# qc-tum/TNC

Measured on NVIDIA H100. Metric: pairwise contractions/sec (effective ZGEMM TFLOP/s in zgemm_tflops), higher is better.
Workload: dtype f64

## Files before the change

tnc_b200/csrc/crt.cu:

```cuda
#include "internal.h"
#include "sm90.h"
#include <cuda.h>
#include <algorithm>
#include <cmath>
#include <cstdio>
#include <cstdlib>

namespace tncb {

constexpr int CRT_MAX_MOD = 20;
static const int kModuli[CRT_MAX_MOD] = {256, 253, 251, 249, 247, 245, 241, 239, 233, 229,
                                         227, 223, 211, 199, 197, 193, 191, 181, 179, 173};
constexpr int CRT_BT = 128;
constexpr int CRT_BKB = WG_BKB;
#ifndef CRT_RING3_STAGES
#define CRT_RING3_STAGES 3
#endif
#ifndef CRT_RING3_BK
#define CRT_RING3_BK 128
#endif
#ifndef CRT_RING4_STAGES
#define CRT_RING4_STAGES 5
#endif
#ifndef CRT_RING4_BK
// ... 65 lines not shown
    T.inv_mod[i] = 1.0 / (double)m;
    T.rho1[i] = std::ldexp((double)q, -CRT_G);
    T.rho2[i] = std::ldexp((double)rem / (double)m, -CRT_G);
  }
  T.p_scaled = (double)std::ldexp(P, -(bits_a + bits_b));
}

int crt_export_tables(int nmod, int* moduli, double* rho1, double* rho2, double* log2_product) {
  CrtTables T;
  crt_make_tables(nmod, 0, 0, T);
  for (int i = 0; i < nmod; i++) {
    if (moduli) moduli[i] = T.mod[i];
    if (rho1) rho1[i] = T.rho1[i];
    if (rho2) rho2[i] = T.rho2[i];
  }
  if (log2_product) *log2_product = crt_log2_product(nmod);
  return TNCB_OK;
}

constexpr int RES_ROWS_C = 32, RES_K_C = 128;
constexpr int kExpNonFinite = 0x7fffffff;
constexpr int kExpMin = -1000;

__device__ __forceinline__ int crt_exp_from_bits(unsigned long long bits) {
  const int field = (int)(bits >> 52) & 0x7ff;
  if (field == 0x7ff) return kExpNonFinite;
  if (field == 0) return bits == 0ull ? 0 : kExpMin;
  return max(field - 1022, kExpMin);
}

__device__ __forceinline__ void crt_tile_coord(int e, int lk, int& r, int& k) {
  const int lane = e & 31, blk = e >> 5;
  const int kb = blk & ((128 >> lk) - 1), rb = blk >> (7 - lk);
  k = (kb << lk) + (lane & ((1 << lk) - 1));
  r = (rb << (5 - lk)) + (lane >> lk);
}

__global__ void __launch_bounds__(256)
crt_rowmax_kernel(const double2* __restrict__ src, const long long* __restrict__ off_row, const long long* __restrict__ off_k,
                  long long rows, long long K, int lk, unsigned long long* __restrict__ rowmax) {
  __shared__ unsigned long long s_max[RES_ROWS_C];
  __shared__ long long s_offr[RES_ROWS_C], s_offk[RES_K_C];
  const long long row0 = (long long)blockIdx.x * RES_ROWS_C, k0 = (long long)blockIdx.y * RES_K_C;
  const int tid = threadIdx.x;
  if (tid < RES_ROWS_C) { s_max[tid] = 0ull; s_offr[tid] = row0 + tid < rows ? __ldg(off_row + row0 + tid) : -1; }
  else if (tid >= 128) { const int k = tid - 128; s_offk[k] = k0 + k < K ? __ldg(off_k + k0 + k) : -1; }
  __syncthreads();
  unsigned long long mv[RES_ROWS_C * RES_K_C / 256];
#pragma unroll
  for (int it = 0; it < RES_ROWS_C * RES_K_C / 256; it++) {
    int r, k;
    crt_tile_coord(it * 256 + tid, lk, r, k);
    const long long orow = s_offr[r], ok = s_offk[k];
    mv[it] = 0ull;
    if (orow >= 0 && ok >= 0) {
      const double2 v = __ldg(src + orow + ok);
      mv[it] = max((unsigned long long)__double_as_longlong(fabs(v.x)), (unsigned long long)__double_as_longlong(fabs(v.y)));
    }
  }
  int cur_r = -1;
  unsigned long long cur_m = 0ull;
#pragma unroll
  for (int it = 0; it < RES_ROWS_C * RES_K_C / 256; it++) {
    int r, k;
    crt_tile_coord(it * 256 + tid, lk, r, k);
    unsigned long long m = mv[it];
    for (int d = 1; d < (1 << lk); d <<= 1) m = max(m, __shfl_xor_sync(0xffffffffu, m, d));
    if (r != cur_r) {
      if (cur_m && (tid & ((1 << lk) - 1)) == 0) atomicMax(&s_max[cur_r], cur_m);
      cur_r = r; cur_m = 0ull;
    }
    cur_m = max(cur_m, m);
  }
  if (cur_m && (tid & ((1 << lk) - 1)) == 0) atomicMax(&s_max[cur_r], cur_m);
  __syncthreads();
  if (tid < RES_ROWS_C && row0 + tid < rows && s_max[tid] != 0ull) atomicMax(rowmax + row0 + tid, s_max[tid]);
}

__device__ __forceinline__ int crt_fix_byte(int s, int m) {
  if (s > 127) s -= m;
  else if (s < -128) s += m;
  return s;
}
constexpr int RES_ROWS = RES_ROWS_C, RES_K = RES_K_C, RES_RS = RES_K + RES_K / 8 + 1;
template <int COMPS, bool KARA>
__global__ void __launch_bounds__(256, 3)
crt_residue_kernel(const double2* __restrict__ src, const long long* __restrict__ off_row, const long long* __restrict__ off_k,
                   long long rows, long long K, long long rowsP, long long Kp, const unsigned long long* __restrict__ rowmax, int bits, int lk,
                   const __grid_constant__ CrtTables T, int8_t* __restrict__ planes) {
  extern __shared__ __align__(16) unsigned char res_smem_raw[];
  double2* tile = reinterpret_cast<double2*>(res_smem_raw);
  __shared__ double s_scale[RES_ROWS];
  __shared__ long long s_offr[RES_ROWS], s_offk[RES_K];
  __shared__ double s_inv[CRT_MAX_MOD];
  __shared__ int s_mod[CRT_MAX_MOD];
  const long long row0 = (long long)blockIdx.x * RES_ROWS, k0 = (long long)blockIdx.y * RES_K;
  const int tid = threadIdx.x;
  const double two_a = scalbn(1.0, bits);
  if (tid >= 64 && tid < 64 + CRT_MAX_MOD) { s_inv[tid - 64] = T.inv_mod[tid - 64]; s_mod[tid - 64] = T.mod[tid - 64]; }
  if (tid < RES_ROWS) {
    const long long r = row0 + tid;
    const int e = r < rows ? crt_exp_from_bits(rowmax[r]) : 0;
    s_scale[tid] = (e == kExpNonFinite) ? 0.0 : scalbn(1.0, -e);
    s_offr[tid] = r < rows ? __ldg(off_row + r) : -1;
  } else if (tid >= 128) {
    const int k = tid - 128;
    s_offk[k] = k0 + k < K ? __ldg(off_k + k0 + k) : -1;
  }
  __syncthreads();
  double2 vv[RES_ROWS * RES_K / 256];
#pragma unroll
  for (int it = 0; it < RES_ROWS * RES_K / 256; it++) {
    int r, k;
    crt_tile_coord(it * 256 + tid, lk, r, k);
    const long long orow = s_offr[r], ok = s_offk[k];
    vv[it] = make_double2(0.0, 0.0);
    if (orow >= 0 && ok >= 0) vv[it] = __ldg(src + orow + ok);
  }
#pragma unroll
  for (int it = 0; it < RES_ROWS * RES_K / 256; it++) {
    int r, k;
    crt_tile_coord(it * 256 + tid, lk, r, k);
    const double sc = s_scale[r];
    double2 v = vv[it];
    v.x = trunc(v.x * sc * two_a);
    v.y = trunc(v.y * sc * two_a);
    if (sc == 0.0) { v.x = 0.0; v.y = 0.0; }
    tile[r * RES_RS + k + (k >> 3)] = v;
  }
  __syncthreads();
  const double RMAGIC = 6755399441055744.0;
  const long long plane_stride = rowsP * Kp;
  const int g = tid & 31;
  const int nmod = T.nmod;
#pragma unroll 1
  for (int pass = 0; pass < RES_ROWS / 8; pass++) {
    const int r = (tid >> 5) + 8 * pass;
    if (row0 + r >= rows) return;
    double xr[4], xi[4];
    int lr[4], li[4];
#pragma unroll
    for (int j = 0; j < 4; j++) {
      const double2 v = tile[r * RES_RS + g * 4 + j + (g >> 1)];
      xr[j] = v.x; xi[j] = v.y;
      lr[j] = (int)__double2ll_rn(v.x); li[j] = (int)__double2ll_rn(v.y);
    }
    int8_t* dst = planes + (row0 + r) * Kp + k0 + g * 4;
#pragma unroll 1
    for (int i = 0; i < nmod; i++) {
      const int m = s_mod[i];
      const double inv = s_inv[i];
      uint32_t wr = 0, wi = 0, ws = 0;
#pragma unroll
      for (int j = 0; j < 4; j++) {
        const int qr = __double2loint(fma(xr[j], inv, RMAGIC));
        const int qi = __double2loint(fma(xi[j], inv, RMAGIC));
        const int rr = lr[j] - qr * m, ri = li[j] - qi * m;
        constexpr uint32_t sel[4] = {0x3214u, 0x3240u, 0x3410u, 0x4210u};
        wr = __byte_perm(wr, (uint32_t)rr, sel[j]);
        wi = __byte_perm(wi, (uint32_t)ri, sel[j]);
        if (KARA) ws = __byte_perm(ws, (uint32_t)crt_fix_byte(rr + ri, m), sel[j]);
      }
      uint32_t* d = reinterpret_cast<uint32_t*>(dst + (long long)i * (KARA ? 3 : COMPS) * plane_stride);
      const long long ps = plane_stride / 4;
      if (KARA) {
        d[0] = wr; d[ps] = wi; d[2 * ps] = ws;
      } else if (COMPS == 2) {
        d[0] = wr; d[ps] = wi;
      } else {
        d[0] = __vneg4(wi); d[ps] = wr; d[2 * ps] = wi;
      }
    }
  }
}

struct CrtGemmArgs {
  int8_t* R;
  int Np, Mp;
  int tiles_n, tiles_m, tile_m;
  int nmod, nkc, kb_per_chunk, num_kb;
  int total_items;
  int group;
  int negmod[CRT_MAX_MOD];
  int magic[CRT_MAX_MOD];
};

struct CrtItem { int mod_i, prod, kc, n0, m0; };
template <bool KARA>
__device__ __forceinline__ CrtItem crt_decode(const CrtGemmArgs& p, int item) {
  const int tiles = p.tiles_n * p.tiles_m;
  const int mk = item / tiles, t = item - mk * tiles;
  CrtItem it;
  const int mp = mk / p.nkc;
  it.kc = mk - mp * p.nkc;
  it.mod_i = KARA ? mp / 3 : mp; it.prod = KARA ? mp - it.mod_i * 3 : 0;
  const int per_band = p.group * p.tiles_m;
  const int band = t / per_band, first = band * p.group;
  const int gsize = min(p.group, p.tiles_n - first);
  const int r = t - band * per_band;
  it.n0 = (first + r % gsize) * CRT_BT;
  it.m0 = (r / gsize) * p.tile_m;
  return it;
}

template <bool KARA>
__global__ void __launch_bounds__(WG_THREADS, 1)
crt_gemm_kernel(const __grid_constant__ CUtensorMap mapB, const __grid_constant__ CUtensorMap mapA,
                const __grid_constant__ CrtGemmArgs p) {
  constexpr int STAGES = CrtRing<KARA>::STAGES, BK = CrtRing<KARA>::BK, SUB = CRT_BKB / BK;
  using Stage = typename CrtRing<KARA>::Stage;
  extern __shared__ __align__(1024) uint8_t crt_smem_raw[];
  uint8_t* smem = reinterpret_cast<uint8_t*>((reinterpret_cast<uintptr_t>(crt_smem_raw) + 1023) & ~(uintptr_t)1023);
  __shared__ uint64_t full_bar[STAGES], empty_bar[STAGES];
  const int wg = threadIdx.x >> 7, tid = threadIdx.x & 127;

  if (threadIdx.x == 0) {
    for (int s = 0; s < STAGES; s++) { wg_mbar_init(&full_bar[s], 1); wg_mbar_init(&empty_bar[s], 2); }
    asm volatile("fence.mbarrier_init.release.cluster;" ::: "memory");
  }
  __syncthreads();

  if (wg == 0) {
    wg_setmaxnreg_producer();
    if (tid != 0) return;
    int it = 0;
    for (int item = blockIdx.x; item < p.total_items; item += gridDim.x) {
      const CrtItem w = crt_decode<KARA>(p, item);
      const int kb0 = w.kc * p.kb_per_chunk, kb1 = min(p.num_kb, kb0 + p.kb_per_chunk);
      const int rowB = (KARA ? w.mod_i * 3 + w.prod : w.mod_i * 2) * p.Np + w.n0;
      const int rowA = (KARA ? w.mod_i * 3 + w.prod : w.mod_i * 3) * p.Mp + w.m0;
      for (int ks = kb0 * SUB; ks < kb1 * SUB; ks++, it++) {
        uint8_t* st = wg_produce_begin<STAGES, KARA, BK>(smem, full_bar, empty_bar, it);
        uint64_t* bar = &full_bar[it % STAGES];
        const int kx = ks * BK;
        uint8_t* a = st + Stage::A;
        wg_tma_2d(&mapB, bar, st, kx, rowB);
        if (KARA) {
          wg_tma_2d(&mapA, bar, a, kx, rowA);
          wg_tma_2d(&mapA, bar, a + Stage::TILE, kx, rowA + WG_ROWS);
        } else {
          wg_tma_2d(&mapB, bar, st + Stage::B1, kx, rowB + p.Np);
          wg_tma_2d(&mapA, bar, a, kx, rowA);
          wg_tma_2d(&mapA, bar, a + Stage::TILE, kx, rowA + p.Mp);
          wg_tma_2d(&mapA, bar, a + 2 * Stage::TILE, kx, rowA + 2 * p.Mp);
        }
      }
    }
  } else {
    wg_setmaxnreg_consumer();
    const int c = wg - 1, wq = tid >> 5, lane = tid & 31;
    const int q = lane & 3;
    const bool q0 = q & 1, q1 = q & 2;
    WgRing<STAGES, KARA, BK> ring{smem, full_bar, empty_bar};
    uint32_t acc[128];
#pragma unroll
    for (int i = 0; i < 128; i++) acc[i] = 0u;
    for (int item = blockIdx.x; item < p.total_items; item += gridDim.x) {
      const CrtItem w = crt_decode<KARA>(p, item);
      const int kb0 = w.kc * p.kb_per_chunk, kb1 = min(p.num_kb, kb0 + p.kb_per_chunk);
      bool first = true;
      for (int ks = kb0 * SUB; ks < kb1 * SUB; ks++) ring.mma_stage(acc, c, first, tid == 0);
      ring.drain(tid == 0);
      const int negm = p.negmod[w.mod_i], magic = p.magic[w.mod_i];
      int8_t* row_base[2];
#pragma unroll
      for (int h = 0; h < 2; h++) {
        const long long n = (long long)w.n0 + c * 64 + wq * 16 + (lane >> 2) + 8 * h;
        row_base[h] = KARA ? p.R + ((long long)((w.mod_i * p.nkc + w.kc) * 3 + w.prod) * p.Np + n) * p.Mp + w.m0
                           : p.R + ((long long)((w.mod_i * p.nkc + w.kc) * 2) * p.Np + n) * p.Mp + w.m0;
      }
#pragma unroll
      for (int i = 0; i < 4; i++) {
#pragma unroll
        for (int h = 0; h < 2; h++) {
          uint32_t x[4];
#pragma unroll
          for (int k = 0; k < 4; k++) {
            uint32_t u = 0;
#pragma unroll
            for (int jj = 0; jj < 2; jj++) {
#pragma unroll
              for (int e = 0; e < 2; e++) {
                const int a = (int)acc[4 * (8 * i + 2 * k + jj) + 2 * h + e];
                int t = __mulhi(a, magic) * negm + a;
                if (t > 127) t += negm;
                u |= (((uint32_t)t & 0xffu) ^ 0x80u) << (8 * (2 * jj + e));
              }
            }
            x[k] = u;
          }
          const uint32_t r0 = __shfl_xor_sync(0xffffffffu, q0 ? x[0] : x[1], 1);
          const uint32_t r1 = __shfl_xor_sync(0xffffffffu, q0 ? x[2] : x[3], 1);
          const uint32_t a0 = q0 ? r0 : x[0], a1 = q0 ? x[1] : r0;
          const uint32_t b0 = q0 ? r1 : x[2], b1 = q0 ? x[3] : r1;
          const uint32_t g0 = __shfl_xor_sync(0xffffffffu, q1 ? a0 : b0, 2);
          const uint32_t g1 = __shfl_xor_sync(0xffffffffu, q1 ? a1 : b1, 2);
          const uint32_t k0 = q1 ? b0 : a0, k1 = q1 ? b1 : a1;
          const uint32_t y0 = q1 ? g0 : k0, y1 = q1 ? g1 : k1, y2 = q1 ? k0 : g0, y3 = q1 ? k1 : g1;
          const uint4 v = make_uint4(__byte_perm(y0, y1, 0x5410), __byte_perm(y2, y3, 0x5410),
                                     __byte_perm(y0, y1, 0x7632), __byte_perm(y2, y3, 0x7632));
          const int cc = 4 * i + q;
          int8_t* dst = KARA ? row_base[h] + cc * 16
                             : row_base[h] + (i >= 2 ? (long long)p.Np * p.Mp : 0LL) + (cc & 7) * 16;
          *reinterpret_cast<uint4*>(dst) = v;
        }
      }
    }
  }
}

struct CrtReconArgs {
  const int8_t* R;
  double2* C;
  const unsigned long long* max_n;
  const unsigned long long* max_m;
  long long rows, cols, ldc;
  long long Np, Mp;
  int nkc;
};

template <bool ONE_CHUNK, bool KARA>
__global__ void __launch_bounds__(256, KARA ? 3 : 4)
crt_reconstruct_kernel(const __grid_constant__ CrtReconArgs a, const __grid_constant__ CrtTables T) {
  constexpr int NPR = KARA ? 3 : 2, RB = 8;
  const long long cols4 = a.Mp >> 2;
  const long long idx = (long long)blockIdx.x * blockDim.x + threadIdx.x;
  const long long n = idx / cols4, m4 = (idx - n * cols4) * 4;
  if (n >= a.rows || m4 >= a.cols) return;
  double s1r[4], s2r[4], s1i[4], s2i[4];
#pragma unroll
  for (int j = 0; j < 4; j++) { s1r[j] = s2r[j] = s1i[j] = s2i[j] = 0.0; }
  const long long plane = a.Np * a.Mp;
  const int8_t* base = a.R + n * a.Mp + m4;
  const double bias = 4503599627370496.0 + (KARA ? 256.0 : 128.0) * (double)a.nkc;
  const double bias_i = 4503599627370496.0 + (KARA ? 384.0 : 128.0) * (double)a.nkc;
  const int nmod = T.nmod;
#pragma unroll 1
  for (int i0 = 0; i0 < nmod; i0 += RB) {
    uint32_t w[RB][NPR];
    if (ONE_CHUNK) {
#pragma unroll
      for (int u = 0; u < RB; u++) {
        if (i0 + u < nmod) {
#pragma unroll
          for (int p = 0; p < NPR; p++) w[u][p] = __ldg(reinterpret_cast<const uint32_t*>(base + (long long)((i0 + u) * NPR + p) * plane));
        }
      }
    }
#pragma unroll
    for (int u = 0; u < RB; u++) {
      const int i = i0 + u;
      if (i >= nmod) break;
      uint32_t ur[4], ui[4];
#pragma unroll
      for (int j = 0; j < 4; j++) { ur[j] = 0; ui[j] = 0; }
      for (int c = 0; c < (ONE_CHUNK ? 1 : a.nkc); c++) {
        uint32_t x[NPR];
        if (ONE_CHUNK) {
#pragma unroll
          for (int p = 0; p < NPR; p++) x[p] = w[u][p];
        } else {
          const int8_t* pk = base + (long long)((i * a.nkc + c) * NPR) * plane;
#pragma unroll
          for (int p = 0; p < NPR; p++) x[p] = __ldg(reinterpret_cast<const uint32_t*>(pk + p * plane));
        }
#pragma unroll
        for (int j = 0; j < 4; j++) {
          const uint32_t k1 = __byte_perm(x[0], 0, 0x4440 + j), k2 = __byte_perm(x[1], 0, 0x4440 + j);
          if (KARA) {
            ur[j] += 256u + k1 - k2;
            ui[j] += 512u + __byte_perm(x[NPR - 1], 0, 0x4440 + j) - k1 - k2;
          } else {
            ur[j] += k1; ui[j] += k2;
          }
        }
      }
      const double r1 = T.rho1[i], r2 = T.rho2[i];
#pragma unroll
      for (int j = 0; j < 4; j++) {
        const double dr = __hiloint2double(0x43300000, (int)ur[j]) - bias;
        const double di = __hiloint2double(0x43300000, (int)ui[j]) - bias_i;
        s1r[j] = fma(dr, r1, s1r[j]); s2r[j] = fma(dr, r2, s2r[j]);
        s1i[j] = fma(di, r1, s1i[j]); s2i[j] = fma(di, r2, s2i[j]);
      }
    }
  }
  const int en = crt_exp_from_bits(a.max_n[n]);
  double2* dst = a.C + n * a.ldc + m4;
  const double RMAGIC = 6755399441055744.0;
#pragma unroll
  for (int j = 0; j < 4; j++) {
    if (m4 + j >= a.cols) break;
    const int em = crt_exp_from_bits(a.max_m[m4 + j]);
    double2 out;
    if (en == kExpNonFinite || em == kExpNonFinite) {
      out = make_double2(__longlong_as_double(0x7ff8000000000000LL), __longlong_as_double(0x7ff8000000000000LL));
    } else {
      const double qr = ((s1r[j] + s2r[j]) + RMAGIC) - RMAGIC;
      const double qi = ((s1i[j] + s2i[j]) + RMAGIC) - RMAGIC;
      const double fr = (s1r[j] - qr) + s2r[j], fi = (s1i[j] - qi) + s2i[j];
      out = make_double2(scalbn(fr * T.p_scaled, en + em), scalbn(fi * T.p_scaled, en + em));
    }
    __stcs(dst + j, out);
  }
}

typedef CUresult (*EncodeTiledFn)(CUtensorMap*, CUtensorMapDataType, cuuint32_t, void*, const cuuint64_t*, const cuuint64_t*,
                                  const cuuint32_t*, const cuuint32_t*, CUtensorMapInterleave, CUtensorMapSwizzle,
                                  CUtensorMapL2promotion, CUtensorMapFloatOOBfill);
static EncodeTiledFn get_encode() {
  static EncodeTiledFn fn = nullptr;
  static bool tried = false;
  if (!tried) {
    tried = true;
    cudaDriverEntryPointQueryResult q;
    void* p = nullptr;
    if (cudaGetDriverEntryPoint("cuTensorMapEncodeTiled", &p, cudaEnableDefault, &q) == cudaSuccess) fn = (EncodeTiledFn)p;
  }
  return fn;
}
template <int BK>
int wg_make_map(CUtensorMap* m, void* ptr, uint64_t rows, uint64_t kbytes) {
  static_assert(BK == 128 || BK == 64, "SWIZZLE_128B or SWIZZLE_64B");
  EncodeTiledFn enc = get_encode();
  if (!enc) return fail(TNCB_ERR_CUDA, "cuTensorMapEncodeTiled is not available");
  cuuint64_t dims[2] = {kbytes, rows};
  cuuint64_t strides[1] = {kbytes};
  cuuint32_t box[2] = {(cuuint32_t)BK, (cuuint32_t)WG_ROWS};
  cuuint32_t estr[2] = {1, 1};
  CUresult r = enc(m, CU_TENSOR_MAP_DATA_TYPE_UINT8, 2, ptr, dims, strides, box, estr, CU_TENSOR_MAP_INTERLEAVE_NONE,
                   BK == 128 ? CU_TENSOR_MAP_SWIZZLE_128B : CU_TENSOR_MAP_SWIZZLE_64B, CU_TENSOR_MAP_L2_PROMOTION_L2_256B,
                   CU_TENSOR_MAP_FLOAT_OOB_FILL_NONE);
  if (r != CUDA_SUCCESS) return fail(TNCB_ERR_CUDA, "cuTensorMapEncodeTiled failed: " + std::to_string((int)r));
  return TNCB_OK;
}
template int wg_make_map<128>(CUtensorMap*, void*, uint64_t, uint64_t);
template int wg_make_map<64>(CUtensorMap*, void*, uint64_t, uint64_t);

static inline long long round_up_ll(long long x, long long a) { return (x + a - 1) / a * a; }


int launch_k1_crt(tncb_ctx* ctx, const PairPlan& P, const double2* A, const double2* B, double2* C,
                  const long long* offAm, const long long* offBn, const long long* offAk, const long long* offBk) {
  int nmod, bits_a, bits_b;
  const int want = ctx->crt_tol > 0.0 ? crt_bits_for_tolerance(P.K, ctx->crt_tol) : ctx->crt_bits;
  crt_choose(P.K, want, ctx->crt_nmod_force, &nmod, &bits_a, &bits_b);
  CrtTables T;
  crt_make_tables(nmod, bits_a, bits_b, T);
  cudaStream_t st = ctx->stream;
  const long long Kp = round_up_ll(P.K, CRT_BKB);
  const int num_kb = (int)(Kp / CRT_BKB);
  const int ctas_max = std::max(1, ctx->sm_count);
  const bool kara = ctx->crt_products == 3 || (ctx->crt_products == 0 && Kp >= ctx->crt_kara_min_k);
  const int TM = kara ? 2 * CRT_BT : CRT_BT;
  const int NPB = kara ? 3 : 2, NPR = kara ? 3 : 2;
  const long long tiles_total = round_up_ll(P.N, CRT_BT) / CRT_BT * (round_up_ll(P.M, TM) / TM);
  int nkc = (int)((Kp + CRT_KCHUNK_MAX - 1) / CRT_KCHUNK_MAX);
  {
    const long long items = tiles_total * nmod * (kara ? 3 : 1);
    const long long want = ctas_max;
    if (items * nkc < want) nkc = (int)std::min<long long>((want + items - 1) / items, std::max(1, num_kb / 8));
    nkc = std::max(1, std::min(nkc, 32));
  }
  int kb_per_chunk = (num_kb + nkc - 1) / nkc;
  nkc = (num_kb + kb_per_chunk - 1) / kb_per_chunk;
  if ((long long)kb_per_chunk * CRT_BKB > CRT_KCHUNK_MAX) return fail(TNCB_ERR_UNSUPPORTED, "K too long for the int8 engine");

  const size_t budget = ctx->crt_ws_bytes;
  long long pn = round_up_ll(P.N, CRT_BT), pm = round_up_ll(P.M, TM);
  auto ws_bytes = [&](long long n_, long long m_) {
    return (size_t)nmod * (size_t)Kp * (size_t)(NPB * n_ + 3 * m_) + (size_t)nmod * nkc * NPR * (size_t)n_ * (size_t)m_;
  };
  while (ws_bytes(pn, pm) > budget && (pm > TM || pn > CRT_BT)) {
    if (pm >= pn && pm > TM) pm = round_up_ll(pm / 2, TM);
    else if (pn > CRT_BT) pn = round_up_ll(pn / 2, CRT_BT);
    else pm = round_up_ll(pm / 2, TM);
  }
  const size_t bytesB = (size_t)nmod * NPB * pn * Kp, bytesA = (size_t)nmod * 3 * pm * Kp;
  const size_t bytesR = (size_t)nmod * nkc * NPR * pn * pm;
  const size_t bytesE = (size_t)(pn + pm) * sizeof(unsigned long long);
  void *pb = nullptr, *pa = nullptr, *pr = nullptr, *pe = nullptr;
  int rc;
  if ((rc = ctx->arena.alloc(bytesB, &pb))) return rc;
  if ((rc = ctx->arena.alloc(bytesA, &pa))) { ctx->arena.free(pb, bytesB); return rc; }
  if ((rc = ctx->arena.alloc(bytesR, &pr))) { ctx->arena.free(pb, bytesB); ctx->arena.free(pa, bytesA); return rc; }
  if ((rc = ctx->arena.alloc(bytesE, &pe))) { ctx->arena.free(pb, bytesB); ctx->arena.free(pa, bytesA); ctx->arena.free(pr, bytesR); return rc; }
  auto cleanup = [&]() { ctx->arena.free(pb, bytesB); ctx->arena.free(pa, bytesA); ctx->arena.free(pr, bytesR); ctx->arena.free(pe, bytesE); };
  unsigned long long* max_n = (unsigned long long*)pe;
  unsigned long long* max_m = max_n + pn;

  static bool attr_done_dev[64] = {false};
  bool& attr_done = attr_done_dev[ctx->device & 63];
  const int smem_gemm4 = CrtRing<false>::SMEM, smem_gemm3 = CrtRing<true>::SMEM;
  const int smem_res = RES_ROWS * RES_RS * (int)sizeof(double2);
  if (!attr_done) {
    cudaError_t e = cudaFuncSetAttribute(crt_gemm_kernel<false>, cudaFuncAttributeMaxDynamicSharedMemorySize, smem_gemm4);
    if (e == cudaSuccess) e = cudaFuncSetAttribute(crt_gemm_kernel<true>, cudaFuncAttributeMaxDynamicSharedMemorySize, smem_gemm3);
    if (e == cudaSuccess) e = cudaFuncSetAttribute(crt_residue_kernel<2, false>, cudaFuncAttributeMaxDynamicSharedMemorySize, smem_res);
    if (e == cudaSuccess) e = cudaFuncSetAttribute(crt_residue_kernel<3, false>, cudaFuncAttributeMaxDynamicSharedMemorySize, smem_res);
    if (e == cudaSuccess) e = cudaFuncSetAttribute(crt_residue_kernel<2, true>, cudaFuncAttributeMaxDynamicSharedMemorySize, smem_res);
    if (e == cudaSuccess) e = cudaFuncSetAttribute(crt_residue_kernel<3, true>, cudaFuncAttributeMaxDynamicSharedMemorySize, smem_res);
    if (e != cudaSuccess) { cleanup(); return fail(TNCB_ERR_CUDA, cudaGetErrorString(e)); }
    attr_done = true;
  }
  auto lane_split = [](const LegList& kl, bool k_is_b, const LegList& fl) {
    auto p2 = [](long long d) { int b = 0; while ((2LL << b) <= d && b < 5) b++; return b; };
    const long long ks = kl.n ? (k_is_b ? kl.sb[kl.n - 1] : kl.sa[kl.n - 1]) : (1LL << 62);
    const long long fs = fl.n ? fl.sa[fl.n - 1] : (1LL << 62);
    if (ks <= fs) return kl.n ? p2(kl.dim[kl.n - 1]) : 0;
    return 0;
  };
  const int lk_b = lane_split(P.k, true, P.n), lk_a = lane_split(P.k, false, P.m);
  ctx->last_int8_ops = 0.0; ctx->last_nmod = nmod; ctx->last_products = kara ? 3 : 4;
  bool timed = false;

  for (long long n0 = 0; n0 < P.N; n0 += pn) {
    const long long nrows = std::min(pn, P.N - n0);
    const long long Np = round_up_ll(nrows, CRT_BT);
    if (Np != nrows) cudaMemsetAsync(pb, 0, (size_t)nmod * NPB * Np * Kp, st);
    cudaMemsetAsync(max_n, 0, (size_t)nrows * sizeof(unsigned long long), st);
    {
      dim3 g((unsigned)((nrows + RES_ROWS - 1) / RES_ROWS), (unsigned)(Kp / RES_K));
      crt_rowmax_kernel<<<g, 256, 0, st>>>(B, offBn + n0, offBk, nrows, P.K, lk_b, max_n);
      if (kara) crt_residue_kernel<2, true><<<g, 256, smem_res, st>>>(B, offBn + n0, offBk, nrows, P.K, Np, Kp, max_n, bits_b, lk_b, T, (int8_t*)pb);
      else crt_residue_kernel<2, false><<<g, 256, smem_res, st>>>(B, offBn + n0, offBk, nrows, P.K, Np, Kp, max_n, bits_b, lk_b, T, (int8_t*)pb);
    }
    ctx->launches += 2;
    CUtensorMap mapB;
    if ((rc = kara ? wg_make_map<CrtRing<true>::BK>(&mapB, pb, (uint64_t)nmod * NPB * Np, (uint64_t)Kp)
                   : wg_make_map<CrtRing<false>::BK>(&mapB, pb, (uint64_t)nmod * NPB * Np, (uint64_t)Kp))) { cleanup(); return rc; }
    for (long long m0 = 0; m0 < P.M; m0 += pm) {
      const long long mcols = std::min(pm, P.M - m0);
      const long long Mp = round_up_ll(mcols, TM);
      if (Mp != mcols) cudaMemsetAsync(pa, 0, (size_t)nmod * 3 * Mp * Kp, st);
      cudaMemsetAsync(max_m, 0, (size_t)mcols * sizeof(unsigned long long), st);
      {
        dim3 g((unsigned)((mcols + RES_ROWS - 1) / RES_ROWS), (unsigned)(Kp / RES_K));
        crt_rowmax_kernel<<<g, 256, 0, st>>>(A, offAm + m0, offAk, mcols, P.K, lk_a, max_m);
        if (kara) crt_residue_kernel<3, true><<<g, 256, smem_res, st>>>(A, offAm + m0, offAk, mcols, P.K, Mp, Kp, max_m, bits_a, lk_a, T, (int8_t*)pa);
        else crt_residue_kernel<3, false><<<g, 256, smem_res, st>>>(A, offAm + m0, offAk, mcols, P.K, Mp, Kp, max_m, bits_a, lk_a, T, (int8_t*)pa);
      }
      ctx->launches += 2;
      CUtensorMap mapA;
      if ((rc = kara ? wg_make_map<CrtRing<true>::BK>(&mapA, pa, (uint64_t)nmod * 3 * Mp, (uint64_t)Kp)
                     : wg_make_map<CrtRing<false>::BK>(&mapA, pa, (uint64_t)nmod * 3 * Mp, (uint64_t)Kp))) { cleanup(); return rc; }
      CrtGemmArgs g;
      g.R = (int8_t*)pr; g.Np = (int)Np; g.Mp = (int)Mp;
      g.tiles_n = (int)(Np / CRT_BT); g.tiles_m = (int)(Mp / TM); g.tile_m = TM;
      g.nmod = nmod; g.nkc = nkc; g.kb_per_chunk = kb_per_chunk; g.num_kb = num_kb;
      const long long items = (long long)g.tiles_n * g.tiles_m * nmod * nkc * (kara ? 3 : 1);
      if (items > 0x7fffffffLL) { cleanup(); return fail(TNCB_ERR_UNSUPPORTED, "too many work items"); }
      g.total_items = (int)items;
      const long long bt_tile_bytes = (long long)CRT_BT * Kp * (kara ? 1 : 2);
      g.group = (int)std::max<long long>(1, std::min<long long>(g.tiles_n, ctx->l2_bytes / 2 / bt_tile_bytes));
      for (int i = 0; i < CRT_MAX_MOD; i++) { g.negmod[i] = -T.mod[i]; g.magic[i] = T.magic[i]; }
      const unsigned grid = (unsigned)std::min<long long>(ctas_max, items);
      const double ops = 2.0 * (kara ? 3.0 : 4.0) * (double)nmod * (double)Np * (double)Mp * (double)Kp;
      const bool time_this = ctx->time_gemm == 2 || (ctx->time_gemm == 1 && !timed);
      if (time_this) gemm_timer_begin(ctx);
      if (kara) crt_gemm_kernel<true><<<grid, WG_THREADS, smem_gemm3, st>>>(mapB, mapA, g);
      else crt_gemm_kernel<false><<<grid, WG_THREADS, smem_gemm4, st>>>(mapB, mapA, g);
      cudaError_t e = cudaGetLastError();
      if (time_this) { gemm_timer_end(ctx, ops); timed = true; }
      if (e != cudaSuccess) { cleanup(); return fail(TNCB_ERR_CUDA, std::string("crt_gemm_kernel launch: ") + cudaGetErrorString(e)); }
      ctx->last_int8_ops += ops;
      CrtReconArgs r;
      r.R = (const int8_t*)pr; r.C = C + n0 * P.M + m0; r.max_n = max_n; r.max_m = max_m;
      r.rows = nrows; r.cols = mcols; r.ldc = P.M; r.Np = Np; r.Mp = Mp; r.nkc = nkc;
      const long long threads = nrows * (Mp / 4);
      const unsigned rg = (unsigned)((threads + 255) / 256);
      if (kara) {
        if (nkc == 1) crt_reconstruct_kernel<true, true><<<rg, 256, 0, st>>>(r, T);
        else crt_reconstruct_kernel<false, true><<<rg, 256, 0, st>>>(r, T);
      } else {
        if (nkc == 1) crt_reconstruct_kernel<true, false><<<rg, 256, 0, st>>>(r, T);
        else crt_reconstruct_kernel<false, false><<<rg, 256, 0, st>>>(r, T);
      }
      ctx->launches += 2;
    }
  }
  ctx->engine_count[4]++;
  cudaError_t e = cudaGetLastError();
  cleanup();
  if (e != cudaSuccess) return fail(TNCB_ERR_CUDA, std::string("K1' (CRT) launch: ") + cudaGetErrorString(e));
  return TNCB_OK;
}

}
```

tnc_b200/csrc/internal.h:

```cpp
#pragma once
#include <cstdint>
#include <cstddef>
#include <string>
#include <vector>
#include <map>
#include <cuda.h>
#include <cuda_runtime.h>
#include "../../include/tncb.h"

namespace tncb {

constexpr int kMaxLegs = 64;
constexpr int kMaxGroups = 40;

struct LegList {
  int n;
  int _pad;
  long long dim[kMaxGroups];
  long long sa[kMaxGroups];
  long long sb[kMaxGroups];
};

struct PairPlan {
  std::vector<uint64_t> out_legs, out_dims;
  long long M = 1, N = 1, K = 1;
  LegList m{}, n{}, k{};
  int kernel_class = 0;
  bool k2_big_is_a = true;
  bool a_kfast = false, b_kfast = true;
  double flops() const { return 8.0 * (double)M * (double)N * (double)K; }
  double bytes() const { return 16.0 * ((double)M * K + (double)K * N + (double)M * N); }
};

int plan_pair(int n_a, const uint64_t* a_legs, const uint64_t* a_dims,
              int n_b, const uint64_t* b_legs, const uint64_t* b_dims, PairPlan& plan);

void set_error(const std::string& msg);
int fail(int status, const std::string& msg);

struct Slab { char* base; size_t size; std::map<size_t, size_t> free_by_off; };

struct Arena {
  std::vector<Slab> slabs;
  size_t capacity_limit = 0;
  size_t reserved = 0, live = 0, peak = 0;
  size_t next_slab = (size_t)256 << 20;
  int alloc(size_t bytes, void** out);
  void free(void* p, size_t bytes);
  void release_all();
  size_t trim();
};

}

struct tncb_tensor {
  double2* ptr = nullptr;
  int rank = 0;
  uint64_t dims[tncb::kMaxLegs];
  uint64_t elems = 1;
  size_t bytes = 0;
  bool owned = true;
};

struct NcclApi;

struct tncb_ctx {
  int device = 0;
  cudaStream_t stream = nullptr;
  tncb::Arena arena;
  uint64_t launches = 0;
  int oz_slices = 8;
  int oz_engine = 0;
  long long oz_min_tiles = 96, oz_min_k = 1536;
  int crt_bits = 53; double crt_tol = 0.0; int crt_nmod_force = 0;
  long long crt_min_k = 256; double crt_min_mnk = 268435456.0;
  size_t crt_ws_bytes = (size_t)12 << 30;
  double last_int8_ops = 0.0; int last_nmod = 0; int last_products = 0;
  int crt_products = 0;
  long long crt_kara_min_k = 2048;
  uint64_t engine_count[8] = {0, 0, 0, 0, 0, 0, 0, 0};
  int time_gemm = 0; cudaEvent_t gemm_ev0 = nullptr, gemm_ev1 = nullptr; bool gemm_ev_valid = false;
  std::vector<cudaEvent_t> gemm_pool; size_t gemm_used = 0; std::vector<double> gemm_ops;
  int sm_count = 132;
  long long l2_bytes = 50LL << 20;
  void* stage_host = nullptr; size_t stage_bytes = 0;
  long long* tab = nullptr; size_t tab_elems = 0;
  bool tab_valid = false; tncb::LegList tab_m{}, tab_n{}, tab_k{};
  double2* partial = nullptr; size_t partial_elems = 0;
  double2* partial_override = nullptr; size_t partial_override_elems = 0;
  void* nccl_comm = nullptr; int world = 1, rank = 0;
  struct HostSlot { void* buf[3] = {nullptr, nullptr, nullptr}; size_t bytes[3] = {0, 0, 0};
                    cudaEvent_t in_done = nullptr, comp_done = nullptr, out_done = nullptr; bool busy = false; };
  HostSlot host_slot[3]; uint64_t host_jobs = 0;
  cudaStream_t h2d_stream = nullptr, d2h_stream = nullptr;
  std::vector<struct tncb_plan*> plans;
  struct CachedPlan { std::vector<uint64_t> key; struct tncb_plan* plan; };
  std::vector<CachedPlan> plan_cache;
  std::vector<struct tncb_angles*> angle_maps;
};

extern "C" void tncb_plan_release_device_state(struct tncb_plan* plan);
namespace tncb { void angles_release(struct tncb_angles* a, tncb_ctx* ctx); }

namespace tncb {
int launch_pair(tncb_ctx* ctx, const PairPlan& p, const double2* A, const double2* B, double2* C,
                int count = 1, long long stride = 0);
int launch_permute(tncb_ctx* ctx, const double2* in, double2* out, int rank,
                   const uint64_t* in_dims, const int* perm);
int launch_conj(tncb_ctx* ctx, double2* data, uint64_t elems);
int launch_add(tncb_ctx* ctx, double2* dst, const double2* src, uint64_t elems);
int ensure_tab(tncb_ctx* ctx, size_t elems);
int launch_k1_ozaki(tncb_ctx* ctx, const PairPlan& p, const double2* A, const double2* B, double2* C, int S,
                    const long long* offAm, const long long* offBn, const long long* offAk, const long long* offBk);

int launch_k1_crt(tncb_ctx* ctx, const PairPlan& p, const double2* A, const double2* B, double2* C,
                  const long long* offAm, const long long* offBn, const long long* offAk, const long long* offBk);
void crt_choose(long long K, int want_bits, int nmod_force, int* nmod, int* bits_a, int* bits_b);
int crt_bits_for_tolerance(long long K, double tol);
int crt_export_tables(int nmod, int* moduli, double* rho1, double* rho2, double* log2_product);

void gemm_timer_begin(tncb_ctx* ctx);
void gemm_timer_end(tncb_ctx* ctx, double ops);

int ensure_partial(tncb_ctx* ctx, size_t elems);
size_t k0_partial_elems(int sm_count, const PairPlan& p);

constexpr int kBatchGroups = 8;
struct CompactLegs { int n; int _pad; long long dim[kBatchGroups]; long long sa[kBatchGroups]; long long sb[kBatchGroups]; };
struct K0BatchItem {
  long long offA, offB, offC;
  long long M, N, K;
  int G, _pad;
  CompactLegs m, n, k;
};
bool k0_batch_eligible(int sm_count, const PairPlan& p);
int k0_batch_fill(int sm_count, const PairPlan& p, K0BatchItem* item);
int launch_k0_batch(tncb_ctx* ctx, const K0BatchItem* d_items, const int* d_block_start, int n_items, int total_blocks, char* ws,
                    int count = 1, long long stride = 0);

constexpr int kGradGroups = 8;
struct GradItem {
  long long src;
  long long dst;
  long long elems;
  int n, _pad;
  long long dim[kGradGroups];
  long long st[kGradGroups];
};
constexpr int kGradThreads = 256;
int launch_grad_gather(tncb_ctx* ctx, const GradItem* d_items, const long long* d_block_start, int n_items,
                       long long total_blocks, const char* ws, double2* out);
int launch_grad_gather_batch(tncb_ctx* ctx, const GradItem* d_items, const long long* d_block_start, int n_items,
                             long long total_blocks, const char* ws, long long stride, int n, double2* rows,
                             long long row_elems, double2* sum);

constexpr int kSliceGroups = 8, kSliceLegs = 8;
struct SliceItem {
  long long slot;
  long long full;
  long long elems;
  int n, ns;
  int from_scratch, _pad;
// ... 64 lines not shown
```

tnc_b200/csrc/runtime.cu:

```cuda
#include "internal.h"
#include <algorithm>
#include <cstdio>
#include <cstdlib>
#include <cstring>
#include <cmath>

namespace tncb {

static inline size_t round_up(size_t x, size_t a) { return (x + a - 1) / a * a; }

int Arena::alloc(size_t bytes, void** out) {
  bytes = round_up(std::max<size_t>(bytes, 256), 256);
  for (Slab& s : slabs) {
    for (auto it = s.free_by_off.begin(); it != s.free_by_off.end(); ++it) {
      if (it->second >= bytes) {
        size_t off = it->first, sz = it->second;
        s.free_by_off.erase(it);
        if (sz > bytes) s.free_by_off[off + bytes] = sz - bytes;
        *out = s.base + off;
        live += bytes; peak = std::max(peak, live);
        return TNCB_OK;
      }
    }
  }
// ... 45 lines not shown
  for (Slab& s : slabs) cudaFree(s.base);
  slabs.clear(); reserved = live = 0;
}

size_t Arena::trim() {
  size_t freed = 0;
  for (size_t i = 0; i < slabs.size();) {
    Slab& s = slabs[i];
    if (s.free_by_off.size() == 1 && s.free_by_off.begin()->first == 0 && s.free_by_off.begin()->second == s.size) {
      cudaFree(s.base);
      freed += s.size; reserved -= s.size;
      slabs.erase(slabs.begin() + i);
    } else i++;
  }
  if (slabs.empty()) next_slab = (size_t)256 << 20;
  return freed;
}

void gemm_timer_begin(tncb_ctx* ctx) {
  if (ctx->time_gemm == 1) cudaEventRecord(ctx->gemm_ev0, ctx->stream);
  else if (ctx->time_gemm == 2) {
    if (ctx->gemm_used + 2 > ctx->gemm_pool.size()) {
      cudaEvent_t a, b; cudaEventCreate(&a); cudaEventCreate(&b);
      ctx->gemm_pool.push_back(a); ctx->gemm_pool.push_back(b);
    }
    cudaEventRecord(ctx->gemm_pool[ctx->gemm_used], ctx->stream);
  }
}

void gemm_timer_end(tncb_ctx* ctx, double ops) {
  if (ctx->time_gemm == 1) { cudaEventRecord(ctx->gemm_ev1, ctx->stream); ctx->gemm_ev_valid = true; }
  else if (ctx->time_gemm == 2) {
    cudaEventRecord(ctx->gemm_pool[ctx->gemm_used + 1], ctx->stream);
    ctx->gemm_used += 2; ctx->gemm_ops.push_back(ops);
  }
}

int tensor_new(tncb_ctx* ctx, int rank, const uint64_t* dims, tncb_tensor** out) {
  if (rank < 0 || rank > kMaxLegs) return fail(TNCB_ERR_INVALID, "tensor rank out of range");
  tncb_tensor* t = new tncb_tensor();
  t->rank = rank; t->elems = 1;
  for (int i = 0; i < rank; i++) { t->dims[i] = dims[i]; t->elems *= dims[i]; }
  t->bytes = std::max<size_t>(t->elems * sizeof(double2), 16);
  void* p = nullptr;
  int rc = ctx->arena.alloc(t->bytes, &p);
  if (rc) { delete t; return rc; }
  t->ptr = (double2*)p;
  *out = t;
  return TNCB_OK;
}

}

using namespace tncb;

extern "C" {

int tncb_ctx_create(int device, size_t arena_bytes, tncb_ctx** out) {
  if (!out) return fail(TNCB_ERR_INVALID, "out is null");
  int count = 0;
  cudaError_t e = cudaGetDeviceCount(&count);
  if (e != cudaSuccess || count == 0) {
    cudaGetLastError();
    return fail(TNCB_ERR_CUDA, std::string("no CUDA device available (") + cudaGetErrorString(e) +
                                   "); libtncb200 has no CPU fallback");
  }
  if (device < 0 || device >= count) return fail(TNCB_ERR_INVALID, "device index out of range");
  TNCB_CUDA(cudaSetDevice(device));
  cudaDeviceProp prop;
  TNCB_CUDA(cudaGetDeviceProperties(&prop, device));
  if (prop.major != 9 || prop.minor != 0)
    return fail(TNCB_ERR_CUDA, std::string("device is sm_") + std::to_string(prop.major * 10 + prop.minor) +
                                   ", libtncb200 is built for sm_90a only");
  tncb_ctx* ctx = new tncb_ctx();
  ctx->device = device;
  ctx->sm_count = prop.multiProcessorCount;
  ctx->l2_bytes = prop.l2CacheSize;
  ctx->arena.capacity_limit = arena_bytes;
  if (const char* e = std::getenv("TNCB_OZAKI_SLICES")) ctx->oz_slices = std::max(0, std::min(8, atoi(e)));
  if (const char* e = std::getenv("TNCB_TCGEN05_ENGINE")) ctx->oz_engine = atoi(e) == 1 ? 1 : 0;
  if (const char* e = std::getenv("TNCB_CRT_MODULI")) ctx->crt_nmod_force = std::max(0, std::min(20, atoi(e)));
  if (const char* e = std::getenv("TNCB_CRT_PRODUCTS")) { const int v = atoi(e); ctx->crt_products = (v == 3 || v == 4) ? v : 0; }
  if (const char* e = std::getenv("TNCB_CRT_MIN_K3")) ctx->crt_kara_min_k = std::max(1, atoi(e));
  if (const char* e = std::getenv("TNCB_CRT_WS_GB")) ctx->crt_ws_bytes = (size_t)std::max(1, atoi(e)) << 30;
  cudaError_t se = cudaStreamCreateWithFlags(&ctx->stream, cudaStreamNonBlocking);
  if (se != cudaSuccess) { delete ctx; return fail(TNCB_ERR_CUDA, cudaGetErrorString(se)); }
  cudaMemPool_t pool;
  if (cudaDeviceGetDefaultMemPool(&pool, device) == cudaSuccess) {
    uint64_t thr = UINT64_MAX;
    cudaMemPoolSetAttribute(pool, cudaMemPoolAttrReleaseThreshold, &thr);
  }
  *out = ctx;
  return TNCB_OK;
}

void tncb_ctx_destroy(tncb_ctx* ctx) {
  if (!ctx) return;
  cudaSetDevice(ctx->device);
  cudaStreamSynchronize(ctx->stream);
  for (auto& c : ctx->plan_cache) tncb_plan_destroy(c.plan);
  ctx->plan_cache.clear();
  while (!ctx->plans.empty()) tncb_plan_release_device_state(ctx->plans.back());
  while (!ctx->angle_maps.empty()) tncb::angles_release(ctx->angle_maps.back(), ctx);
  tncb_comm_destroy(ctx);
  if (ctx->tab) cudaFree(ctx->tab);
  if (ctx->partial) cudaFree(ctx->partial);
  if (ctx->stage_host) cudaFreeHost(ctx->stage_host);
  if (ctx->gemm_ev0) { cudaEventDestroy(ctx->gemm_ev0); cudaEventDestroy(ctx->gemm_ev1); }
  for (cudaEvent_t e : ctx->gemm_pool) cudaEventDestroy(e);
  if (ctx->h2d_stream) {
    cudaStreamSynchronize(ctx->h2d_stream); cudaStreamSynchronize(ctx->d2h_stream);
    for (auto& sl : ctx->host_slot) {
      for (int i = 0; i < 3; i++) if (sl.buf[i]) cudaFree(sl.buf[i]);
      cudaEventDestroy(sl.in_done); cudaEventDestroy(sl.comp_done); cudaEventDestroy(sl.out_done);
    }
    cudaStreamDestroy(ctx->h2d_stream); cudaStreamDestroy(ctx->d2h_stream);
  }
  ctx->arena.release_all();
  cudaStreamDestroy(ctx->stream);
  delete ctx;
}

int tncb_ctx_synchronize(tncb_ctx* ctx) {
  if (!ctx) return fail(TNCB_ERR_INVALID, "ctx is null");
  TNCB_CUDA(cudaSetDevice(ctx->device));
  TNCB_CUDA(cudaStreamSynchronize(ctx->stream));
  if (ctx->d2h_stream) {
    TNCB_CUDA(cudaStreamSynchronize(ctx->h2d_stream));
    TNCB_CUDA(cudaStreamSynchronize(ctx->d2h_stream));
    for (auto& sl : ctx->host_slot) sl.busy = false;
  }
  return TNCB_OK;
}

int tncb_contract_pair_host(tncb_ctx* ctx, int n_a, const uint64_t* a_legs, const uint64_t* a_dims, const double* host_a,
                            int n_b, const uint64_t* b_legs, const uint64_t* b_dims, const double* host_b, double* host_c) {
  if (!ctx || !host_a || !host_b || !host_c) return fail(TNCB_ERR_INVALID, "null argument");
  TNCB_CUDA(cudaSetDevice(ctx->device));
  PairPlan P;
  int rc = plan_pair(n_a, a_legs, a_dims, n_b, b_legs, b_dims, P);
  if (rc) return rc;
  size_t ea = 1, eb = 1;
  for (int i = 0; i < n_a; i++) ea *= a_dims[i];
  for (int i = 0; i < n_b; i++) eb *= b_dims[i];
  const size_t need[3] = {std::max<size_t>(ea * 16, 16), std::max<size_t>(eb * 16, 16), std::max<size_t>((size_t)(P.M * P.N) * 16, 16)};
  if (!ctx->h2d_stream) {
    TNCB_CUDA(cudaStreamCreateWithFlags(&ctx->h2d_stream, cudaStreamNonBlocking));
    TNCB_CUDA(cudaStreamCreateWithFlags(&ctx->d2h_stream, cudaStreamNonBlocking));
    for (auto& sl : ctx->host_slot) {
      TNCB_CUDA(cudaEventCreateWithFlags(&sl.in_done, cudaEventDisableTiming));
      TNCB_CUDA(cudaEventCreateWithFlags(&sl.comp_done, cudaEventDisableTiming));
      TNCB_CUDA(cudaEventCreateWithFlags(&sl.out_done, cudaEventDisableTiming));
    }
  }
  tncb_ctx::HostSlot& sl = ctx->host_slot[ctx->host_jobs % 3];
  if (sl.busy) TNCB_CUDA(cudaEventSynchronize(sl.out_done));
  for (int i = 0; i < 3; i++)
    if (sl.bytes[i] < need[i]) {
      if (sl.buf[i]) TNCB_CUDA(cudaFree(sl.buf[i]));
      sl.buf[i] = nullptr; sl.bytes[i] = 0;
      cudaError_t e = cudaMalloc(&sl.buf[i], need[i]);
      if (e != cudaSuccess) { cudaGetLastError(); return fail(TNCB_ERR_OOM, std::string("cudaMalloc (host pipeline): ") + cudaGetErrorString(e)); }
      sl.bytes[i] = need[i];
    }
  TNCB_CUDA(cudaMemcpyAsync(sl.buf[0], host_a, ea * 16, cudaMemcpyHostToDevice, ctx->h2d_stream));
  TNCB_CUDA(cudaMemcpyAsync(sl.buf[1], host_b, eb * 16, cudaMemcpyHostToDevice, ctx->h2d_stream));
// ... 298 lines not shown
```

Measured before the change: 6146.

## Permute A-plane rows so GEMM epilogue stores residues without warp shuffles

The residue kernel now writes the A operand planes with a row permutation inside each 64-row group. This makes the int32 accumulator fragments each lane holds in the GEMM epilogue map to contiguous output bytes, so the epilogue can pack residues with byte_perm and packed 16-bit adds and store 16 bytes per lane, dropping the shuffle transpose. A fallback path without the permutation (env TNCB_CRT_PLAIN_AT) stores 2-byte chunks. This adds template variants and depends on the consumer reading the permuted row order consistently.

Result: faster. 6283, median of 6 (+2.2%).

```diff
diff --git a/tnc_b200/csrc/crt.cu b/tnc_b200/csrc/crt.cu
--- a/tnc_b200/csrc/crt.cu
+++ b/tnc_b200/csrc/crt.cu
@@ -171,12 +171,17 @@
   else if (s < -128) s += m;
   return s;
 }
+__host__ __device__ __forceinline__ long long crt_at_plane_row(long long m) {
+  const int u = (int)(m & 63);
+  return (m & ~63LL) | (((u >> 1) & 7) << 3) | ((u >> 4) << 1) | (u & 1);
+}
+
 constexpr int RES_ROWS = RES_ROWS_C, RES_K = RES_K_C, RES_RS = RES_K + RES_K / 8 + 1;
 template <int COMPS, bool KARA>
 __global__ void __launch_bounds__(256, 3)
 crt_residue_kernel(const double2* __restrict__ src, const long long* __restrict__ off_row, const long long* __restrict__ off_k,
                    long long rows, long long K, long long rowsP, long long Kp, const unsigned long long* __restrict__ rowmax, int bits, int lk,
-                   const __grid_constant__ CrtTables T, int8_t* __restrict__ planes) {
+                   int at_perm, const __grid_constant__ CrtTables T, int8_t* __restrict__ planes) {
   extern __shared__ __align__(16) unsigned char res_smem_raw[];
   double2* tile = reinterpret_cast<double2*>(res_smem_raw);
   __shared__ double s_scale[RES_ROWS];
@@ -234,7 +239,8 @@
       xr[j] = v.x; xi[j] = v.y;
       lr[j] = (int)__double2ll_rn(v.x); li[j] = (int)__double2ll_rn(v.y);
     }
-    int8_t* dst = planes + (row0 + r) * Kp + k0 + g * 4;
+    const long long prow = (COMPS == 3 && at_perm) ? crt_at_plane_row(row0 + r) : row0 + r;
+    int8_t* dst = planes + prow * Kp + k0 + g * 4;
 #pragma unroll 1
     for (int i = 0; i < nmod; i++) {
       const int m = s_mod[i];
@@ -292,7 +298,22 @@
   return it;
 }
 
-template <bool KARA>
+__device__ __forceinline__ uint32_t crt_acc_residue(uint32_t acc, int negm, int magic) {
+  const int a = (int)acc;
+  int t = __mulhi(a, magic) * negm + a;
+  asm("{\n\t.reg .pred p;\n\tsetp.gt.s32 p, %0, 127;\n\t@p add.s32 %0, %0, %1;\n\t}" : "+r"(t) : "r"(negm));
+  return (uint32_t)t;
+}
+__device__ __forceinline__ uint32_t crt_acc_offset_pair(uint32_t acc0, uint32_t acc1, int negm, uint32_t negm2, int magic) {
+  const int a0 = (int)acc0, a1 = (int)acc1;
+  const int t0 = __mulhi(a0, magic) * negm + a0, t1 = __mulhi(a1, magic) * negm + a1;
+  uint32_t x, r;
+  asm("add.s16x2 %0, %1, %2;" : "=r"(x) : "r"(__byte_perm((uint32_t)t0, (uint32_t)t1, 0x5410)), "r"(0xff80ff80u));
+  asm("{\n\t.reg .b32 y;\n\tadd.s16x2 y, %1, %2;\n\tmax.u16x2 %0, %1, y;\n\t}" : "=r"(r) : "r"(x), "r"(negm2));
+  return r;
+}
+
+template <bool KARA, bool PERM>
 __global__ void __launch_bounds__(WG_THREADS, 1)
 crt_gemm_kernel(const __grid_constant__ CUtensorMap mapB, const __grid_constant__ CUtensorMap mapA,
                 const __grid_constant__ CrtGemmArgs p) {
@@ -339,7 +360,6 @@
     wg_setmaxnreg_consumer();
     const int c = wg - 1, wq = tid >> 5, lane = tid & 31;
     const int q = lane & 3;
-    const bool q0 = q & 1, q1 = q & 2;
     WgRing<STAGES, KARA, BK> ring{smem, full_bar, empty_bar};
     uint32_t acc[128];
 #pragma unroll
@@ -358,40 +378,36 @@
         row_base[h] = KARA ? p.R + ((long long)((w.mod_i * p.nkc + w.kc) * 3 + w.prod) * p.Np + n) * p.Mp + w.m0
                            : p.R + ((long long)((w.mod_i * p.nkc + w.kc) * 2) * p.Np + n) * p.Mp + w.m0;
       }
-#pragma unroll
-      for (int i = 0; i < 4; i++) {
-#pragma unroll
-        for (int h = 0; h < 2; h++) {
-          uint32_t x[4];
-#pragma unroll
-          for (int k = 0; k < 4; k++) {
-            uint32_t u = 0;
-#pragma unroll
-            for (int jj = 0; jj < 2; jj++) {
-#pragma unroll
-              for (int e = 0; e < 2; e++) {
-                const int a = (int)acc[4 * (8 * i + 2 * k + jj) + 2 * h + e];
-                int t = __mulhi(a, magic) * negm + a;
-                if (t > 127) t += negm;
-                u |= (((uint32_t)t & 0xffu) ^ 0x80u) << (8 * (2 * jj + e));
-              }
+      const long long im_off = KARA ? 0LL : (long long)p.Np * p.Mp;
+      if (PERM) {
+        const uint32_t negm2 = ((uint32_t)negm & 0xffffu) * 0x10001u;
+#pragma unroll
+        for (int s = 0; s < 4; s++) {
+#pragma unroll
+          for (int h = 0; h < 2; h++) {
+            uint32_t v[4];
+#pragma unroll
+            for (int x = 0; x < 4; x++) {
+              const int j = 8 * s + 2 * x;
+              v[x] = __byte_perm(crt_acc_offset_pair(acc[4 * j + 2 * h], acc[4 * j + 2 * h + 1], negm, negm2, magic),
+                                 crt_acc_offset_pair(acc[4 * j + 4 + 2 * h], acc[4 * j + 4 + 2 * h + 1], negm, negm2, magic),
+                                 0x6420);
             }
-            x[k] = u;
+            int8_t* dst = KARA ? row_base[h] + 64 * s + 16 * q : row_base[h] + (s >= 2 ? im_off : 0LL) + 64 * (s & 1) + 16 * q;
+            *reinterpret_cast<uint4*>(dst) = make_uint4(v[0], v[1], v[2], v[3]);
           }
-          const uint32_t r0 = __shfl_xor_sync(0xffffffffu, q0 ? x[0] : x[1], 1);
-          const uint32_t r1 = __shfl_xor_sync(0xffffffffu, q0 ? x[2] : x[3], 1);
-          const uint32_t a0 = q0 ? r0 : x[0], a1 = q0 ? x[1] : r0;
-          const uint32_t b0 = q0 ? r1 : x[2], b1 = q0 ? x[3] : r1;
-          const uint32_t g0 = __shfl_xor_sync(0xffffffffu, q1 ? a0 : b0, 2);
-          const uint32_t g1 = __shfl_xor_sync(0xffffffffu, q1 ? a1 : b1, 2);
-          const uint32_t k0 = q1 ? b0 : a0, k1 = q1 ? b1 : a1;
-          const uint32_t y0 = q1 ? g0 : k0, y1 = q1 ? g1 : k1, y2 = q1 ? k0 : g0, y3 = q1 ? k1 : g1;
-          const uint4 v = make_uint4(__byte_perm(y0, y1, 0x5410), __byte_perm(y2, y3, 0x5410),
-                                     __byte_perm(y0, y1, 0x7632), __byte_perm(y2, y3, 0x7632));
-          const int cc = 4 * i + q;
-          int8_t* dst = KARA ? row_base[h] + cc * 16
-                             : row_base[h] + (i >= 2 ? (long long)p.Np * p.Mp : 0LL) + (cc & 7) * 16;
-          *reinterpret_cast<uint4*>(dst) = v;
+        }
+      } else {
+#pragma unroll
+        for (int j = 0; j < 32; j++) {
+#pragma unroll
+          for (int h = 0; h < 2; h++) {
+            const uint32_t u = __byte_perm(crt_acc_residue(acc[4 * j + 2 * h], negm, magic),
+                                           crt_acc_residue(acc[4 * j + 2 * h + 1], negm, magic), 0x0040) ^ 0x8080u;
+            const int col = 8 * j + 2 * q;
+            int8_t* dst = KARA ? row_base[h] + col : row_base[h] + (col >= 128 ? im_off : 0LL) + (col & 127);
+            *reinterpret_cast<uint16_t*>(dst) = (uint16_t)u;
+          }
         }
       }
     }
@@ -541,6 +557,7 @@
   const int num_kb = (int)(Kp / CRT_BKB);
   const int ctas_max = std::max(1, ctx->sm_count);
   const bool kara = ctx->crt_products == 3 || (ctx->crt_products == 0 && Kp >= ctx->crt_kara_min_k);
+  const int at_perm = ctx->crt_plain_at ? 0 : 1;
   const int TM = kara ? 2 * CRT_BT : CRT_BT;
   const int NPB = kara ? 3 : 2, NPR = kara ? 3 : 2;
   const long long tiles_total = round_up_ll(P.N, CRT_BT) / CRT_BT * (round_up_ll(P.M, TM) / TM);
@@ -583,8 +600,10 @@
   const int smem_gemm4 = CrtRing<false>::SMEM, smem_gemm3 = CrtRing<true>::SMEM;
   const int smem_res = RES_ROWS * RES_RS * (int)sizeof(double2);
   if (!attr_done) {
-    cudaError_t e = cudaFuncSetAttribute(crt_gemm_kernel<false>, cudaFuncAttributeMaxDynamicSharedMemorySize, smem_gemm4);
-    if (e == cudaSuccess) e = cudaFuncSetAttribute(crt_gemm_kernel<true>, cudaFuncAttributeMaxDynamicSharedMemorySize, smem_gemm3);
+    cudaError_t e = cudaFuncSetAttribute(crt_gemm_kernel<false, true>, cudaFuncAttributeMaxDynamicSharedMemorySize, smem_gemm4);
+    if (e == cudaSuccess) e = cudaFuncSetAttribute(crt_gemm_kernel<true, true>, cudaFuncAttributeMaxDynamicSharedMemorySize, smem_gemm3);
+    if (e == cudaSuccess) e = cudaFuncSetAttribute(crt_gemm_kernel<false, false>, cudaFuncAttributeMaxDynamicSharedMemorySize, smem_gemm4);
+    if (e == cudaSuccess) e = cudaFuncSetAttribute(crt_gemm_kernel<true, false>, cudaFuncAttributeMaxDynamicSharedMemorySize, smem_gemm3);
     if (e == cudaSuccess) e = cudaFuncSetAttribute(crt_residue_kernel<2, false>, cudaFuncAttributeMaxDynamicSharedMemorySize, smem_res);
     if (e == cudaSuccess) e = cudaFuncSetAttribute(crt_residue_kernel<3, false>, cudaFuncAttributeMaxDynamicSharedMemorySize, smem_res);
     if (e == cudaSuccess) e = cudaFuncSetAttribute(crt_residue_kernel<2, true>, cudaFuncAttributeMaxDynamicSharedMemorySize, smem_res);
@@ -611,8 +630,8 @@
     {
       dim3 g((unsigned)((nrows + RES_ROWS - 1) / RES_ROWS), (unsigned)(Kp / RES_K));
       crt_rowmax_kernel<<<g, 256, 0, st>>>(B, offBn + n0, offBk, nrows, P.K, lk_b, max_n);
-      if (kara) crt_residue_kernel<2, true><<<g, 256, smem_res, st>>>(B, offBn + n0, offBk, nrows, P.K, Np, Kp, max_n, bits_b, lk_b, T, (int8_t*)pb);
-      else crt_residue_kernel<2, false><<<g, 256, smem_res, st>>>(B, offBn + n0, offBk, nrows, P.K, Np, Kp, max_n, bits_b, lk_b, T, (int8_t*)pb);
+      if (kara) crt_residue_kernel<2, true><<<g, 256, smem_res, st>>>(B, offBn + n0, offBk, nrows, P.K, Np, Kp, max_n, bits_b, lk_b, at_perm, T, (int8_t*)pb);
+      else crt_residue_kernel<2, false><<<g, 256, smem_res, st>>>(B, offBn + n0, offBk, nrows, P.K, Np, Kp, max_n, bits_b, lk_b, at_perm, T, (int8_t*)pb);
     }
     ctx->launches += 2;
     CUtensorMap mapB;
@@ -626,8 +645,8 @@
       {
         dim3 g((unsigned)((mcols + RES_ROWS - 1) / RES_ROWS), (unsigned)(Kp / RES_K));
         crt_rowmax_kernel<<<g, 256, 0, st>>>(A, offAm + m0, offAk, mcols, P.K, lk_a, max_m);
-        if (kara) crt_residue_kernel<3, true><<<g, 256, smem_res, st>>>(A, offAm + m0, offAk, mcols, P.K, Mp, Kp, max_m, bits_a, lk_a, T, (int8_t*)pa);
-        else crt_residue_kernel<3, false><<<g, 256, smem_res, st>>>(A, offAm + m0, offAk, mcols, P.K, Mp, Kp, max_m, bits_a, lk_a, T, (int8_t*)pa);
+        if (kara) crt_residue_kernel<3, true><<<g, 256, smem_res, st>>>(A, offAm + m0, offAk, mcols, P.K, Mp, Kp, max_m, bits_a, lk_a, at_perm, T, (int8_t*)pa);
+        else crt_residue_kernel<3, false><<<g, 256, smem_res, st>>>(A, offAm + m0, offAk, mcols, P.K, Mp, Kp, max_m, bits_a, lk_a, at_perm, T, (int8_t*)pa);
       }
       ctx->launches += 2;
       CUtensorMap mapA;
@@ -647,8 +666,13 @@
       const double ops = 2.0 * (kara ? 3.0 : 4.0) * (double)nmod * (double)Np * (double)Mp * (double)Kp;
       const bool time_this = ctx->time_gemm == 2 || (ctx->time_gemm == 1 && !timed);
       if (time_this) gemm_timer_begin(ctx);
-      if (kara) crt_gemm_kernel<true><<<grid, WG_THREADS, smem_gemm3, st>>>(mapB, mapA, g);
-      else crt_gemm_kernel<false><<<grid, WG_THREADS, smem_gemm4, st>>>(mapB, mapA, g);
+      if (at_perm) {
+        if (kara) crt_gemm_kernel<true, true><<<grid, WG_THREADS, smem_gemm3, st>>>(mapB, mapA, g);
+        else crt_gemm_kernel<false, true><<<grid, WG_THREADS, smem_gemm4, st>>>(mapB, mapA, g);
+      } else {
+        if (kara) crt_gemm_kernel<true, false><<<grid, WG_THREADS, smem_gemm3, st>>>(mapB, mapA, g);
+        else crt_gemm_kernel<false, false><<<grid, WG_THREADS, smem_gemm4, st>>>(mapB, mapA, g);
+      }
       cudaError_t e = cudaGetLastError();
       if (time_this) { gemm_timer_end(ctx, ops); timed = true; }
       if (e != cudaSuccess) { cleanup(); return fail(TNCB_ERR_CUDA, std::string("crt_gemm_kernel launch: ") + cudaGetErrorString(e)); }
diff --git a/tnc_b200/csrc/internal.h b/tnc_b200/csrc/internal.h
--- a/tnc_b200/csrc/internal.h
+++ b/tnc_b200/csrc/internal.h
@@ -78,6 +78,7 @@
   double last_int8_ops = 0.0; int last_nmod = 0; int last_products = 0;
   int crt_products = 0;
   long long crt_kara_min_k = 2048;
+  bool crt_plain_at = false;
   uint64_t engine_count[8] = {0, 0, 0, 0, 0, 0, 0, 0};
   int time_gemm = 0; cudaEvent_t gemm_ev0 = nullptr, gemm_ev1 = nullptr; bool gemm_ev_valid = false;
   std::vector<cudaEvent_t> gemm_pool; size_t gemm_used = 0; std::vector<double> gemm_ops;
diff --git a/tnc_b200/csrc/runtime.cu b/tnc_b200/csrc/runtime.cu
--- a/tnc_b200/csrc/runtime.cu
+++ b/tnc_b200/csrc/runtime.cu
@@ -151,6 +151,7 @@
   if (const char* e = std::getenv("TNCB_CRT_MODULI")) ctx->crt_nmod_force = std::max(0, std::min(20, atoi(e)));
   if (const char* e = std::getenv("TNCB_CRT_PRODUCTS")) { const int v = atoi(e); ctx->crt_products = (v == 3 || v == 4) ? v : 0; }
   if (const char* e = std::getenv("TNCB_CRT_MIN_K3")) ctx->crt_kara_min_k = std::max(1, atoi(e));
+  if (const char* e = std::getenv("TNCB_CRT_PLAIN_AT")) ctx->crt_plain_at = atoi(e) != 0;
   if (const char* e = std::getenv("TNCB_CRT_WS_GB")) ctx->crt_ws_bytes = (size_t)std::max(1, atoi(e)) << 30;
   cudaError_t se = cudaStreamCreateWithFlags(&ctx->stream, cudaStreamNonBlocking);
   if (se != cudaSuccess) { delete ctx; return fail(TNCB_ERR_CUDA, cudaGetErrorString(se)); }
```
